# YuQiao0303/PointDreamer

Measured on AMD Instinct MI355X. Metric: shapes/hour (30k-pt cloud, 8x256^2 views, DDNM) on MI355X, higher is better.
Workload: dtype f16 (f32 accumulate; f32 GroupNorm/softmax statistics, f32 geometry); 1 GPU; configs[2]: synthetic 30k-point sphere shape, 8x256^2 views, texture_gen_method='DDNM_inpaint' (100 DDNM steps, 552.8M-param guided-diffusion UNet, random-init weights), NBF [21], atlas 1024^2, complete_unseen_by='unproject', optimize_from=None, hidden-point removal on (device); 4 independent shapes per step, their views batched through the UNet together; parallelism=shapes-parallel x1, views_per_unet_batch=32

## Files before the change

include/pdhip.h:

```cpp
#ifndef PDHIP_H
#define PDHIP_H
#include <stdint.h>
#include <stddef.h>
#ifdef __cplusplus
extern "C" {
#endif

#define PDHIP_OK 0
#define PDHIP_E_ARG (-1)
#define PDHIP_E_HIP (-2)
#define PDHIP_E_STATE (-3)
#define PDHIP_E_NOMEM (-4)
#define PDHIP_E_UNKNOWN_NAME (-5)

int pdhip_version(void);
int pdhip_lab_build(void);
const char* pdhip_last_error(void);

int pdhip_project_points(const float* cam_params, int V, const float* vertices, int Vn,
                         const float* points, int N, int rescale, double padding,
                         float* pos , float* vertice_uvs ,
                         float* uv_centers, float* uv_scales,
                         float* point_uvs , float* point_depths ,
                         uint32_t* minmax_ws, void* stream);
// ... 239 lines not shown
int pdhip_gn_finalize_oct_f32(const float* partA, int Ca, int chunksA, const float* partB, int Cb, int chunksB, int N, int HW, float* stats, void* stream);
int pdhip_conv_ht_f16(const void* x, const void* w_packed, const float* bias, const void* residual, int res_up, void* y, int N, int H, int W, int Cin, int Cout,
                      int Cout_pad, const void* zero_page, float* splitk_ws, long long splitk_ws_floats, float* gn_part, int* gn_chunks, void* stream);
int pdhip_conv_ht_plan(int N, int H, int W, int Cin, int Cout, int Cout_pad, long long splitk_ws_floats, int* routed, int* slabs);
int pdhip_debug_set_conv_ht(int mode, int slabs);
int pdhip_debug_set_rr_gn(int max_width);
int pdhip_debug_set_conv_rr(int mode, int variant, int slabs);
int pdhip_attention_f16(const void* qkv , void* out , int N, int T, int C, int head_dim,
                        void* vt_ws , void* stream);
int pdhip_philox_normal(float* out, long long n, uint64_t seed, uint64_t stream_id, void* stream);
int pdhip_gemv_rows_f32(const float* W, const float* b, const float* x, float* y, int R, int K, int N, int silu_out, void* stream);
int pdhip_timestep_mlp_f32(const float* t, int N, int mc, const float* w0, const float* b0, const float* w2, const float* b2, float* emb_silu,
                           float* tmp, void* stream);
int pdhip_conv_in_f16(const float* x_nchw, const void* Wt, const float* bias, void* Y, int N, int H, int W, int Cout, int Cout_pad, void* im2col_ws,
                      const void* zero_page, void* stream);
int pdhip_bench_copy16(const void* src, void* dst, long long bytes, int blocks, int unroll, void* stream);

#ifdef __cplusplus
}
#endif
#endif
```

pointdreamer_amd/csrc/nn_common.h:

```cpp
#pragma once
#include "common.h"
#include <hip/hip_fp16.h>

namespace pdnn {

typedef _Float16 half_t;
typedef __attribute__((ext_vector_type(8))) _Float16 half8;
typedef __attribute__((ext_vector_type(4))) _Float16 half4;
typedef __attribute__((ext_vector_type(4))) float float4_t;

bool conv3x3_halo_eligible(int N, int H, int W, int Cin, int Cout_pad);
int conv3x3_halo_splits(int N, int H, int W, int Cin, int Cout, int Cout_pad, size_t splitk_ws_floats);
int conv3x3_halo_launch_splits(int N, int H, int W, int Cin, int Cout, int Cout_pad, size_t halo_ws_floats);
int conv3x3_halo(const half_t* X, const half_t* Wt, const float* bias, const half_t* residual, half_t* Y, int N, int H, int W,
                 int Cin, int Cout, int Cout_pad, const half_t* zero_page, hipStream_t s, float* gn_part, int* gn_fused,
                 float* splitk_ws, size_t splitk_ws_floats, const float* apply_table = nullptr, int res_up = 0,
                 int in_up = 0);
int splitk_reduce(const float* partial, int splits, long long M, int Cout, const float* bias, const half_t* residual, half_t* Y,
                  float* gn_part, int hw, hipStream_t s);
extern thread_local int g_force_bk, g_force_stages, g_force_wmw, g_force_splits;
extern thread_local int g_fuse_gn, g_fold_resample, g_fold_finalize, g_fuse_skip, g_fold_skip;
extern thread_local float* g_dbg_splitk_ws; extern thread_local size_t g_dbg_splitk_floats;
int conv_igemm(const half_t* X, const half_t* Wt, const float* bias, const half_t* residual, half_t* Y, int N, int H,
               int W, int Cin, int Cout, int Cout_pad, int taps, const half_t* zero_page, hipStream_t s,
// ... 83 lines not shown
__device__ __forceinline__ float silu_f(float x) { return x * __builtin_amdgcn_rcpf(1.0f + __expf(-x)); }

__device__ __forceinline__ float gn_round_f16(float f) { asm("" : "+v"(f)); return (float)(half_t)f; }
template <bool OUT_F32, bool FILM>
__device__ __forceinline__ float gn_elem(float x, float ga, float gb, float t1, float sh, int silu) {
    float f = __builtin_fmaf(x, ga, gb);
    if (!OUT_F32) f = gn_round_f16(f);
    if (FILM) {
        f = gn_round_f16(f * t1);
        f = gn_round_f16(f + sh);
    }
    if (silu) { f = silu_f(f); if (!OUT_F32) f = gn_round_f16(f); }
    return f;
}


int gn_stats(const half_t* X, int N, int HW, int C, float eps, float* stats, float* ws, size_t ws_floats, hipStream_t s);
struct GnPartsArg { const float* partA; int Ca, chunksA; const float* partB; int Cb, chunksB; float eps; };
int gn_apply(const half_t* X, const float* stats, const float* gamma, const float* beta, const float* film,
             long long film_stride, int N, int H, int W, int C, int silu, int resample, void* Y, int out_f32, hipStream_t s,
             const half_t* XB = nullptr, int Ca = 0,
             half_t* Yraw = nullptr,
             const GnPartsArg* parts = nullptr);
int gn_table(const float* stats, const float* gamma, const float* beta, const float* film, long long film_stride, int N, int C,
             float* table, hipStream_t s);
bool gn_skip_eligible(int N, int HW, int Ca, int C, int Cout, int Cout_pad);
int gn_skip(const half_t* XA, const half_t* XB, int Ca, int C, const float* stats, const float* gamma, const float* beta, const half_t* Wt,
            const float* bias, half_t* H0, half_t* SK, int N, int HW, hipStream_t s);
int resample2x(const half_t* X, int N, int H, int W, int C, int mode, half_t* Y, hipStream_t s);
int concat_channels(const half_t* A, int Ca, const half_t* B, int Cb, long long pixels, half_t* Y, hipStream_t s);

int attention(const half_t* qkv, half_t* out, int N, int T, int C, int D, hipStream_t s, half_t* vt_ws = nullptr);

int conv_in_3x3(const float* x_nchw, const half_t* Wt , const float* bias, half_t* Y,
                int N, int H, int W, int Cout, int Cout_pad, half_t* im2col_ws , const half_t* zero_page, hipStream_t s, float* gn_part = nullptr, int* gn_fused = nullptr);
int head_pack(const float* w, int NO, int C, half_t* wz, hipStream_t s);
int head_gn_silu_conv3x3(const half_t* X, const float* stats, const float* gamma, const float* beta, const half_t* wz,
                         const float* bias, float* y_nchw, int N, int H, int W, int C, int NO, hipStream_t s);
int timestep_mlp(const float* t, int N, int mc, const float* w0, const float* b0, const float* w2, const float* b2,
                 float* emb_silu , float* tmp, hipStream_t s);
int gemv_rows(const float* Wm , const float* b, const float* x , float* y , int R, int K, int N,
              hipStream_t s);

struct DdnmCoef { float sqrt_1m_at, sqrt_at, sqrt_at_next, sigma_t, c1, c2; };
int ddnm_update(float* x , const float* et , int Cet, const float* y,
                const float* mask , const float* eps , unsigned long long seed,
                unsigned long long step, DdnmCoef co, int N, int HW, hipStream_t s, unsigned long long quad0 = 0);
int ddnm_prepare(const float* masked_img, const float* mask, float* y, int N, int HW, hipStream_t s);
int ddnm_finish(const float* x, float* out, long long n, hipStream_t s);
extern thread_local int g_gn_iters;
// ... 6 lines not shown
```

pointdreamer_amd/csrc/nn_misc.hip:

```cpp
#include "nn_common.h"
using namespace pdhip;
namespace pdnn {

__global__ __launch_bounds__(256) void k_im2col_in(const float* __restrict__ x, half_t* __restrict__ A, int H, int W,
                                                   long long pixels) {
    for (long long p = blockIdx.x * (long long)blockDim.x + threadIdx.x; p < pixels; p += (long long)gridDim.x * blockDim.x) {
        const int xx = (int)(p % W), y = (int)((p / W) % H);
        const long long n = p / ((long long)W * H);
        half_t row[32];
#pragma unroll
        for (int k = 27; k < 32; ++k) row[k] = (half_t)0.f;
#pragma unroll
        for (int ky = 0; ky < 3; ++ky)
#pragma unroll
            for (int kx = 0; kx < 3; ++kx) {
                const int yy = y + ky - 1, xc = xx + kx - 1;
                const bool ok = yy >= 0 && yy < H && xc >= 0 && xc < W;
#pragma unroll
                for (int c = 0; c < 3; ++c)
                    row[(ky * 3 + kx) * 3 + c] = ok ? (half_t)x[(((size_t)n * 3 + c) * H + yy) * W + xc] : (half_t)0.f;
            }
        half8* dst = reinterpret_cast<half8*>(A + (size_t)p * 32);
#pragma unroll
        for (int q = 0; q < 4; ++q) {
            half8 v;
#pragma unroll
            for (int e = 0; e < 8; ++e) v[e] = row[q * 8 + e];
            dst[q] = v;
        }
    }
}

int conv_in_3x3(const float* x_nchw, const half_t* Wt, const float* bias, half_t* Y, int N, int H, int W, int Cout, int Cout_pad,
                half_t* im2col_ws, const half_t* zero_page, hipStream_t s, float* gn_part, int* gn_fused) {
    const long long pixels = (long long)N * H * W;
    k_im2col_in<<<(int)std::min<long long>((pixels + 255) / 256, 8192), 256, 0, s>>>(x_nchw, im2col_ws, H, W, pixels);
    PD_LAUNCH_CHECK();
    return conv_igemm(im2col_ws, Wt, bias, nullptr, Y, N, H, W, 32, Cout, Cout_pad, 1, zero_page, s, nullptr, 0, gn_part, gn_fused);
}

#define GEMV_ROWS 128
template <int KI>
__global__ __launch_bounds__(256) void k_gemv_rows(const float* __restrict__ Wm, const float* __restrict__ b,
                                                   const float* __restrict__ x, float* __restrict__ y, int R, int K, int N,
                                                   int silu_out) {
    extern __shared__ __attribute__((aligned(16))) float s_x[];
    const int lane = threadIdx.x & 63, wave = threadIdx.x >> 6;
    const int r0 = blockIdx.x * GEMV_ROWS + wave * (GEMV_ROWS / 4);
    for (int n0 = 0; n0 < N; n0 += 8) {
        const int nb = min(8, N - n0);
// ... 239 lines not shown
    return pdnn::gemv_launch(W, b, x, y, R, K, N, silu_out != 0, as_stream(stream));
}
extern "C" int pdhip_timestep_mlp_f32(const float* t, int N, int mc, const float* w0, const float* b0, const float* w2, const float* b2,
                                      float* emb_silu, float* tmp, void* stream) {
    PD_REQUIRE(t && w0 && b0 && w2 && b2 && emb_silu && tmp, "pdhip_timestep_mlp_f32: null argument");
    PD_REQUIRE(N >= 1 && mc >= 2 && mc % 2 == 0 && mc <= 512, "pdhip_timestep_mlp_f32: N must be positive and mc even, at most 512 (N=%d mc=%d)", N, mc);
    return pdnn::timestep_mlp(t, N, mc, w0, b0, w2, b2, emb_silu, tmp, as_stream(stream));
}
extern "C" int pdhip_conv_in_f16(const float* x_nchw, const void* Wt, const float* bias, void* Y, int N, int H, int W, int Cout, int Cout_pad,
                                 void* im2col_ws, const void* zero_page, void* stream) {
    PD_REQUIRE(x_nchw && Wt && bias && Y && im2col_ws && zero_page, "pdhip_conv_in_f16: null argument");
    PD_REQUIRE(N >= 1 && H >= 1 && W >= 1 && Cout >= 1, "pdhip_conv_in_f16: N, H, W, Cout must be positive");
    return pdnn::conv_in_3x3(x_nchw, (const pdnn::half_t*)Wt, bias, (pdnn::half_t*)Y, N, H, W, Cout, Cout_pad, (pdnn::half_t*)im2col_ws, (const pdnn::half_t*)zero_page,
                             as_stream(stream), nullptr, nullptr);
}
```

pointdreamer_amd/csrc/nn_norm.hip:

```cpp
#include "nn_common.h"
using namespace pdhip;
namespace pdnn {

#define GN_PIX_PER_BLOCK 256

__global__ __launch_bounds__(256) void k_gn_partial(const half_t* __restrict__ X, int HW, int C, float* __restrict__ part) {
    extern __shared__ float s_acc[];
    const int n = blockIdx.y, chunk = blockIdx.x;
    const int opp = C >> 3;
    const int pps = max(1, 256 / opp);
    const int tid = threadIdx.x;
    const int sub = tid / opp, oct = tid - sub * opp;
    const int p0 = chunk * GN_PIX_PER_BLOCK;
    const int p1 = min(HW, p0 + GN_PIX_PER_BLOCK);
    float s[8], q[8];
#pragma unroll
    for (int e = 0; e < 8; ++e) { s[e] = 0.f; q[e] = 0.f; }
    if (sub < pps) {
        for (int oc = oct; oc < opp; oc += 256) {
            for (int p = p0 + sub; p < p1; p += pps) {
                const half8 v = *reinterpret_cast<const half8*>(X + ((size_t)n * HW + p) * C + oc * 8);
#pragma unroll
                for (int e = 0; e < 8; ++e) { const float f = (float)v[e]; s[e] += f; q[e] += f * f; }
            }
// ... 113 lines not shown
            float* row = table + ((size_t)n * (C / 8) + (c >> 3)) * 16;
            row[c & 7] = ga * t1; row[8 + (c & 7)] = gb * t1 + sh;
        }
    }
}
int gn_table(const float* stats, const float* gamma, const float* beta, const float* film, long long film_stride, int N, int C,
             float* table, hipStream_t s) {
    PD_REQUIRE(C % 32 == 0, "gn_table: C %% 32 != 0");
    k_gn_table<<<dim3(cdiv(C, 256), N), 256, 0, s>>>(stats, gamma, beta, film, film_stride, C, table);
    PD_LAUNCH_CHECK();
    return PDHIP_OK;
}


#define GNA_ITERS 8
struct GnParts { const float* a; const float* b; int Ca, Cb, chunksA, chunksB; float eps; };
template <int RES, bool OUT_F32, bool FILM, bool FIN>
__global__ __launch_bounds__(256) void k_gn_apply(const half_t* __restrict__ X, const float* __restrict__ stats,
                                                  const float* __restrict__ gamma, const float* __restrict__ beta,
                                                  const float* __restrict__ film, long long film_stride, int H, int W,
                                                  int C, int silu, void* __restrict__ Yv, const half_t* __restrict__ XB, int Ca, int iters,
                                                  half_t* __restrict__ Yraw, GnParts gp) {
    const int opp = C >> 3, cg = C / 32;
    const int pps = max(1, 256 / opp);
    const int Ho = RES == 1 ? H / 2 : (RES == 2 ? H * 2 : H), Wo = RES == 1 ? W / 2 : (RES == 2 ? W * 2 : W);
    __shared__ double s_fin[FIN ? 512 : 1];
    __shared__ float s_st[FIN ? 64 : 1];
    if (FIN) {
        const int img = blockIdx.y, fs = threadIdx.x / opp, fo = threadIdx.x - fs * opp;
        if (fs < pps) {
            const int oa = gp.Ca >> 3;
            const bool inA = fo < oa;
            const int chunks = inA ? gp.chunksA : gp.chunksB, os = inA ? oa : (gp.Cb >> 3);
            const float2* src = reinterpret_cast<const float2*>(inA ? gp.a : gp.b) + (size_t)img * chunks * os + (inA ? fo : fo - oa);
            double ds = 0.0, dq = 0.0;
#pragma unroll 8
            for (int c = fs; c < chunks; c += pps) { const float2 v = src[(size_t)c * os]; ds += (double)v.x; dq += (double)v.y; }
            s_fin[(fs * opp + fo) * 2] = ds; s_fin[(fs * opp + fo) * 2 + 1] = dq;
        }
        __syncthreads();
        if (threadIdx.x < 32) {
            const int opg = cg >> 3, g = threadIdx.x;
            double ds = 0.0, dq = 0.0;
            for (int k = 0; k < opg; ++k)
                for (int sl = 0; sl < pps; ++sl) { ds += s_fin[(sl * opp + g * opg + k) * 2]; dq += s_fin[(sl * opp + g * opg + k) * 2 + 1]; }
            const double cnt = (double)H * W * cg;
            const double mean = ds / cnt;
            double var = dq / cnt - mean * mean;
            if (var < 0.0) var = 0.0;
            s_st[2 * g] = (float)mean; s_st[2 * g + 1] = (float)(1.0 / sqrt(var + (double)gp.eps));
        }
        __syncthreads();
    }
#ifdef PD_LAB_GN_REV
    const int n = gridDim.y - 1 - blockIdx.y, bx = gridDim.x - 1 - blockIdx.x;
#else
    const int n = blockIdx.y, bx = blockIdx.x;
#endif
    const int sub = threadIdx.x / opp;
    if (sub >= pps) return;
    const int p_begin = bx * (pps * iters), p_end = min(Ho * Wo, p_begin + pps * iters);
    for (int oc = threadIdx.x - sub * opp; oc < opp; oc += 256) {
        const int c0 = oc * 8;
        const bool second = XB != nullptr && c0 >= Ca;
        const half_t* const Xs = second ? XB + (c0 - Ca) : X + c0;
        const int cs = XB == nullptr ? C : (second ? C - Ca : Ca);
        float ga[8], gb[8], t1[8], sh[8];
#pragma unroll
// ... 364 lines not shown
```

pointdreamer_amd/csrc/nn_unet.hip:

```cpp
#include "nn_common.h"
#include <map>
#include <string>
#include <vector>
#include <cmath>
#include <cstring>
using namespace pdhip;
using namespace pdnn;

namespace {

struct ConvW { half_t* w = nullptr; float* b = nullptr; int cin = 0, cout = 0, cout_pad = 0, taps = 0; bool have_w = false, have_b = false;
               half_t* wf = nullptr; half_t* wph = nullptr; bool has_wf = false, has_wph = false; };
struct NormW { float* g = nullptr; float* b = nullptr; int c = 0; bool have_g = false, have_b = false; };
struct ResB { std::string name; int cin, cout, mode; NormW n1, n2; ConvW c1, c2, skip; long long emb_off; bool has_skip; bool have_ew = false, have_eb = false;
              half_t* c2s_w = nullptr; float* c2s_b = nullptr; bool c2s_ready = false; half_t* c2s_wf = nullptr; int hw = 0; bool has_c2s = false, has_c2s_wf = false; };
struct AttB { std::string name; int c; NormW n; ConvW qkv, proj; };
struct Block { int kind; int idx; };

struct Act { half_t* p; int C, H, W; const float* gn_part = nullptr; int gn_chunks = 0; const float* gn_partB = nullptr; int Ca = 0; int gn_chunksB = 0;
             half_t* p2 = nullptr;
             int row = -1, rowB = -1; };

}
namespace pdnn { thread_local int g_fuse_gn = 0; }
namespace pdnn { thread_local int g_fold_resample = 1; }
namespace pdnn { thread_local int g_fold_skip = 1; }
namespace pdnn { thread_local int g_rr_gn = 0; }
namespace pdnn { thread_local int g_fold_finalize = 8; thread_local int g_fold_finalize_chunks = 16; }
namespace pdnn { thread_local int g_fuse_skip = 1; thread_local int g_fuse_skip_min_tiles = 1; }
namespace pdnn { thread_local int g_up_phase = 1; }
namespace {
struct Prof { std::vector<hipEvent_t> ev; std::vector<uint8_t> cls; size_t used = 0; double flops[2] = {0, 0}; bool on = false;
              int period = 1; long long forwards = 0; bool armed = false; };

}

// ... 188 lines not shown
}
ConvPlan plan_conv(const Ctx& c, const Act& x, const ConvW& w, bool want_gn) {
    ConvNeeds nd;
    nd.two_source = x.p2 != nullptr; nd.want_gn = want_gn; nd.have_wf = w.has_wf;
    return conv_plan(c.N, x.H, x.W, w.cin, w.cout, w.cout_pad, w.taps, nd, c.u->splitk_floats);
}

int run_gn_stats(Ctx& c, const Act& x) {
    if (x.gn_part != nullptr && ((x.C / 32) % 8) == 0)
        return gn_finalize_oct(x.gn_part, x.Ca, x.gn_chunks, x.gn_partB, x.C - x.Ca, x.gn_chunksB, c.N, x.H * x.W, 1e-5f, c.u->stats, c.s);
    PD_REQUIRE(x.p2 == nullptr, "unet: a virtual concat needs fused GroupNorm partials of both tensors");
    return gn_stats(x.p, c.N, x.H * x.W, x.C, 1e-5f, c.u->stats, c.u->gn_ws, c.u->gn_ws_floats, c.s);
}

int run_gn(Ctx& c, const Act& x, const NormW& n, const float* film, long long film_stride, int silu, int resample, Act* out,
           half_t* raw_pool = nullptr) {
    *out = Act{nullptr, x.C, 0, 0};
    out->H = resample == 1 ? x.H / 2 : (resample == 2 ? x.H * 2 : x.H);
    out->W = resample == 1 ? x.W / 2 : (resample == 2 ? x.W * 2 : x.W);
    out->p = arena_take(c.u, (size_t)c.N * out->H * out->W * x.C);
    if (!c.go()) return PDHIP_OK;
    PD_REQUIRE(n.have_g && n.have_b, "unet: norm weights not loaded");
#ifdef PD_LAB_SKIP_GN
    if (resample == 0 && x.p2 == nullptr && x.W <= 128 && silu) { out->p = x.p; return PDHIP_OK; }
#endif
    if (x.gn_part != nullptr && ((x.C / 32) % 8) == 0 && (x.C >> 3) <= 256 && g_fold_finalize > 0 &&
        (c.N <= g_fold_finalize || (x.gn_chunks <= g_fold_finalize_chunks && x.gn_chunksB <= g_fold_finalize_chunks))) {
        const GnPartsArg pa{x.gn_part, x.Ca, x.gn_chunks, x.gn_partB, x.C - x.Ca, x.gn_chunksB, 1e-5f};
        return gn_apply(x.p, nullptr, n.g, n.b, film, film_stride, c.N, x.H, x.W, x.C, silu, resample, out->p, 0, c.s, x.p2,
                        x.p2 ? x.Ca : 0, raw_pool, &pa);
    }
    PD_TRY(run_gn_stats(c, x));
    return gn_apply(x.p, c.u->stats, n.g, n.b, film, film_stride, c.N, x.H, x.W, x.C, silu, resample, out->p, 0, c.s, x.p2, x.p2 ? x.Ca : 0,
                    raw_pool);
}

int run_gn_then_conv(Ctx& c, const std::string& name, const ConvPlan& p, const Act& x, const NormW& n, const float* film, long long film_stride,
                     int resample, half_t* raw_pool, const ConvW& w, ConvIn in, Act* out) {
    if (p.takes_apply) {
        if (c.go()) {
            PD_REQUIRE(n.have_g && n.have_b, "unet: norm weights not loaded");
            PD_TRY(run_gn_stats(c, x));
            PD_TRY(gn_table(c.u->stats, n.g, n.b, film, film_stride, c.N, x.C, c.u->ap_table, c.s));
            in.apply_table = c.u->ap_table;
        }
        in.x = &x;
        return run_conv(c, name, p, w, in, out);
    }
    if (p.takes_in_gn) {
        if (c.go()) PD_REQUIRE(n.have_g && n.have_b, "unet: norm weights not loaded");
        const RrIn rr_in{x.p, nullptr, x.C, x.C, 2, n.g, n.b, film, film_stride, x.gn_part, nullptr, x.gn_chunks, 0, 1e-5f};
        in.x = &x; in.rr_in = &rr_in; in.parts_of = &x;
        return run_conv(c, name, p, w, in, out);
    }
    Act h;
    PD_TRY(run_gn(c, x, n, film, film_stride, 1, resample, &h, raw_pool));
    in.x = &h;
    if (x.p2 != nullptr) in.parts_of = &x;
    return run_conv(c, name, p, w, in, out);
}

struct ResPlan {
    bool fuse_skip = false;
    bool fold_down = false;
    bool fold_up = false;
    bool skip_conv = false;
    ConvPlan c1, c2, skip;
};
bool wish_in_gn(const Act& x, const ConvW& w, int W) {
    if (g_rr_gn <= 0 || W > g_rr_gn || x.p2 != nullptr || x.gn_part == nullptr || x.gn_partB != nullptr || ((x.C / 32) % 8) != 0 || w.cin > 1024 ||
        x.C != w.cin) return false;
    const int pps = std::max(1, 256 / (x.C >> 3));
    return (x.gn_chunks + pps - 1) / pps <= PD_RR_MAX_PART_LOADS;
}
bool wish_up_phase(int N, const ResB& rb, int H, int W) {
    if (g_up_phase == 0 || rb.mode != 2 || !rb.c1.has_wph || (H * W) % 256 != 0 ||
        !conv_up2_phase_eligible(N, H, W, rb.c1.cin, rb.c1.cout, rb.c1.cout_pad)) return false;
    if (g_up_phase == 2) return true;
    const long long tiles = (long long)N * H * W / 256 * 4 * (rb.c1.cout_pad / (rb.c1.cout_pad % 256 == 0 ? 256 : 128));
    return tiles >= 128;
}
// ... 3 lines not shown
    const bool lean = !conservative;
    const bool fold = g_fold_resample != 0 && lean && x.p2 == nullptr && !rb.has_skip;
    r.fold_down = fold && rb.mode == 1;
    r.fuse_skip = rb.has_skip && rb.mode == 0 && g_fuse_skip != 0 && rb.skip.taps == 1 && x.C == rb.skip.cin &&
                  gn_skip_eligible(N, x.H * x.W, x.p2 ? x.Ca : x.C, x.C, rb.skip.cout, rb.skip.cout_pad) &&
                  (g_fuse_skip == 2 || (long long)N * x.H * x.W / 128 >= g_fuse_skip_min_tiles) &&
                  (conservative || (x.gn_part != nullptr && ((x.C / 32) % 8) == 0));
    ConvNeeds n1;
    n1.want_gn = true; n1.have_wf = rb.c1.has_wf;
    if (lean && !r.fuse_skip && rb.mode == 0 && x.p2 == nullptr) { n1.apply = g_fuse_gn != 0; n1.in_gn = wish_in_gn(x, rb.c1, x.W); }
    n1.in_up = fold && rb.mode == 2;
    if (lean && x.p2 == nullptr && !rb.has_skip && wish_up_phase(N, rb, x.H, x.W))
        r.c1 = conv_up2_phase_plan(N, Ho, Wo, rb.c1.cin, rb.c1.cout, rb.c1.cout_pad, true);
    else
        r.c1 = conv_plan(N, Ho, Wo, rb.c1.cin, rb.c1.cout, rb.c1.cout_pad, 9, n1, ws_floats);
    Act h1{nullptr, rb.cout, Ho, Wo};
    if (r.c1.gn_chunks > 0) { h1.gn_part = x.gn_part ? x.gn_part : reinterpret_cast<const float*>(&r); h1.gn_chunks = r.c1.gn_chunks; h1.Ca = rb.cout; }
    ConvNeeds n2;
    n2.want_gn = true; n2.have_wf = rb.c2.has_wf;
    if (lean) { n2.apply = g_fuse_gn != 0; n2.in_gn = wish_in_gn(h1, rb.c2, Wo); }
    if (lean && rb.has_skip && !r.fuse_skip && g_fold_skip != 0 && rb.mode == 0 && rb.has_c2s && rb.skip.taps == 1 &&
        (x.p2 == nullptr || (x.Ca % 64 == 0 && (x.C - x.Ca) % 64 == 0))) {
        n2.skip_cs = rb.skip.cin;
        n2.have_wf_skip = rb.has_c2s_wf && (x.p2 == nullptr || (x.Ca % 128 == 0 && (x.C - x.Ca) % 128 == 0));
    }
    r.c2 = conv_plan(N, Ho, Wo, rb.c2.cin, rb.c2.cout, rb.c2.cout_pad, 9, n2, ws_floats);
    r.fold_up = fold && rb.mode == 2 && r.c2.takes_res_up;
    r.skip_conv = rb.has_skip && !r.fuse_skip && !r.c2.takes_skip;
    if (r.skip_conv) {
        ConvNeeds ns;
// ... 16 lines not shown
    if (r.fuse_skip) {
        Act h0{nullptr, x.C, x.H, x.W};
        h0.p = arena_take(c.u, (size_t)c.N * x.H * x.W * x.C);
        sk = Act{nullptr, rb.skip.cout, x.H, x.W};
        sk.p = arena_take(c.u, (size_t)c.N * x.H * x.W * rb.skip.cout);
        if (c.go()) {
            PD_REQUIRE(rb.n1.have_g && rb.n1.have_b && rb.skip.have_w && rb.skip.have_b, "unet: norm / skip weights of %s not loaded", rb.name.c_str());
            PD_TRY(run_gn_stats(c, x));
            PD_TRY(gn_skip(x.p, x.p2, x.p2 ? x.Ca : x.C, x.C, c.u->stats, rb.n1.g, rb.n1.b, rb.skip.w, rb.skip.b, h0.p, sk.p, c.N, x.H * x.W, c.s));
        }
        ConvIn in{&h0};
        in.parts_of = &x; in.note = "gn_skip";
        PD_TRY(run_conv(c, n1, r.c1, rb.c1, in, &h1));
    } else {
        const bool half_res = r.c1.kernel == CONV_UP_PHASE || r.c1.takes_in_up;
        PD_TRY(run_gn_then_conv(c, n1, r.c1, x, rb.n1, nullptr, 0, half_res ? 0 : rb.mode, r.fold_down ? xr.p : nullptr, rb.c1, ConvIn{nullptr}, &h1));
    }
    if (rb.mode != 0 && c.go() && !r.fold_down && !r.fold_up) PD_TRY(resample2x(x.p, c.N, x.H, x.W, x.C, rb.mode, xr.p, c.s));
    if (!r.fuse_skip) sk = r.fold_up ? x : xr;
    if (r.skip_conv) PD_TRY(run_conv(c, rb.name + ".skip_connection", r.skip, rb.skip, ConvIn{&xr}, &sk));
    ConvIn in2{nullptr, r.c2.takes_skip ? nullptr : sk.p, r.fold_up ? 1 : 0};
    in2.skip_src = &x; in2.skip_w = &rb;
    return run_gn_then_conv(c, rb.name + ".out_layers.3", r.c2, h1, rb.n2, film, c.film_stride, 0, nullptr, rb.c2, in2, out);
}

int run_att(Ctx& c, const Act& x, AttB& ab, Act* out) {
    Act xn, qkv, a;
    PD_TRY(run_gn(c, x, ab.n, nullptr, 0, 0, 0, &xn));
    PD_TRY(run_conv(c, ab.name + ".qkv", plan_conv(c, xn, ab.qkv, false), ab.qkv, ConvIn{&xn}, &qkv));
    a = x;
    a.p = arena_take(c.u, (size_t)c.N * x.H * x.W * x.C);
    half_t* vt = arena_take(c.u, (size_t)c.N * x.H * x.W * x.C);
    if (c.go()) {
        const double T = (double)x.H * x.W;
        PD_TRY(prof_begin(c, 4.0 * c.N * T * T * x.C, 1));
        PD_TRY(attention(qkv.p, a.p, c.N, x.H * x.W, x.C, c.u->head, c.s, vt));
        PD_TRY(prof_end(c));
    }
    return run_conv(c, ab.name + ".proj_out", plan_conv(c, a, ab.proj, true), ab.proj, ConvIn{&a, x.p}, out);
}

int run_blocks(Ctx& c, std::vector<Block>& blocks, Act* h, const float* x_nchw) {
    for (Block& b : blocks) {
        Act o;
        if (b.kind == 0) {
            o.C = c.u->mult[0] * c.u->mc; o.H = o.W = c.u->image_size;
            const int cpad = ((o.C + 127) / 128) * 128;
            ConvNeeds nd;
            nd.want_gn = true;
            const ConvPlan p = conv_plan(c.N, o.H, o.W, 32, o.C, cpad, 1, nd, 0);
            o.p = arena_take(c.u, (size_t)c.N * o.H * o.W * o.C);
            half_t* col = arena_take(c.u, (size_t)c.N * o.H * o.W * 32);
            float* part = reinterpret_cast<float*>(arena_take(c.u, (size_t)c.N * ((o.H * o.W + 127) / 128) * (o.C / 8) * 2 * 2));
            if (c.table) { Act in{nullptr, 32, o.H, o.W}; table_row(c, "input_blocks.0.0", p, ConvIn{&in}, &o); adopt_parts(&o, part, p.gn_chunks); }
            if (c.go()) {
                PD_REQUIRE(c.u->have_win && c.u->have_bin, "unet: input conv not loaded");
                int chunks = 0;
                PD_TRY(conv_in_3x3(x_nchw, c.u->w_in, c.u->b_in, o.p, c.N, o.H, o.W, o.C, cpad, col, c.u->zero_page, c.s, part, &chunks));
                PD_REQUIRE(chunks == p.gn_chunks, "unet: input conv: planned for %d partial chunks per image, the launcher left %d", p.gn_chunks, chunks);
                adopt_parts(&o, part, chunks);
            }
// ... 553 lines not shown
    int old = pdnn::g_sk_mode;
    pdnn::g_sk_mode = mode; pdnn::g_sk_tile = tile; pdnn::g_sk_splits = splits;
    return old;
}
extern "C" int pdhip_debug_set_conv_sk_stages(int stages) { int old = pdnn::g_sk_stages; pdnn::g_sk_stages = stages; return old; }
extern "C" int pdhip_debug_set_conv_sk_kgroups(int kg) { int old = pdnn::g_sk_kg; pdnn::g_sk_kg = kg; return old; }
namespace pdnn { extern thread_local int g_attn_nbuf, g_attn_vt, g_attn_qtn; }
extern "C" int pdhip_debug_set_attn(int nbuf, int vt_form, int qtiles) {
    int old = pdnn::g_attn_nbuf | (pdnn::g_attn_vt << 8) | (pdnn::g_attn_qtn << 16);
    pdnn::g_attn_nbuf = nbuf; pdnn::g_attn_vt = vt_form; pdnn::g_attn_qtn = qtiles;
    return old;
}
extern "C" int pdhip_debug_set_conv_sk_order(int order) { int old = pdnn::g_sk_order; pdnn::g_sk_order = order; return old; }
extern "C" int pdhip_debug_set_rr_gn(int max_width) { int old = pdnn::g_rr_gn; pdnn::g_rr_gn = max_width; return old; }
extern "C" int pdhip_debug_set_up_phase(int mode) { int old = pdnn::g_up_phase; pdnn::g_up_phase = mode; return old; }
extern "C" int pdhip_pack_conv_up2_phase_f16(const void* w_packed, int Cin, int Cout_pad, void* w_phase, void* stream) {
    PD_REQUIRE(w_packed && w_phase && Cin > 0 && Cout_pad > 0, "pdhip_pack_conv_up2_phase_f16: bad arguments");
    return conv_up2_phase_pack((const half_t*)w_packed, Cin, Cout_pad, (half_t*)w_phase, as_stream(stream));
}
extern "C" int pdhip_conv3x3_up2_phase_nhwc_f16(const void* x, const void* w_phase, const float* bias, void* y, int N, int H, int W, int Cin, int Cout,
                                                int Cout_pad, const void* zero_page, float* gn_part, void* stream) {
    PD_REQUIRE(x && w_phase && y && zero_page, "pdhip_conv3x3_up2_phase_nhwc_f16: null argument");
    return conv_up2_phase((const half_t*)x, (const half_t*)w_phase, bias, (half_t*)y, N, H, W, Cin, Cout, Cout_pad, (const half_t*)zero_page,
                          as_stream(stream), gn_part, nullptr);
}
extern "C" int pdhip_conv3x3_up2_halo_nhwc_f16(const void* x, const void* w_packed, const float* bias, void* y, int N, int H, int W, int Cin, int Cout,
                                               int Cout_pad, const void* zero_page, void* stream) {
    PD_REQUIRE(x && w_packed && y && zero_page, "pdhip_conv3x3_up2_halo_nhwc_f16: null argument");
    pdnn::ConvNeeds nd;
    nd.in_up = true;
// ... 95 lines not shown
```

pointdreamer_amd/ddnm_inpainting.py:

```python
import ctypes as C
import math
import os

import torch

from . import _lib
from ._lib import ptr, stream, check

_reg = _lib.register
vp, i32, i64, f32, f64, u64 = C.c_void_p, C.c_int, C.c_int64, C.c_float, C.c_double, C.c_uint64
_reg('pdhip_unet_create', C.c_int, [i32, i32, i32, C.POINTER(C.c_int), i32, C.POINTER(C.c_int), i32, i32, i32, i32,
                                    C.POINTER(vp)])
_reg('pdhip_unet_destroy', None, [vp])
_reg('pdhip_unet_arena_bytes', C.c_longlong, [vp])
_reg('pdhip_unet_num_tensors', C.c_int, [vp])
_reg('pdhip_unet_load_tensor', C.c_int, [vp, C.c_char_p, vp, i32, C.POINTER(C.c_int64), i32, vp])
_reg('pdhip_unet_missing_tensors', C.c_int, [vp, C.c_char_p, i32])
_reg('pdhip_unet_forward', C.c_int, [vp, vp, vp, i32, vp, vp])
_reg('pdhip_unet_profile', C.c_int, [vp, i32])
_reg('pdhip_unet_profile_read', C.c_int, [vp, C.POINTER(C.c_double), C.POINTER(C.c_double), C.POINTER(C.c_longlong)])
_reg('pdhip_unet_profile_read_attention', C.c_int, [vp, C.POINTER(C.c_double), C.POINTER(C.c_double), C.POINTER(C.c_longlong)])
_reg('pdhip_ddnm_schedule', C.c_int, [vp, vp, vp, vp, vp])
_reg('pdhip_ddnm_prepare', C.c_int, [vp, vp, vp, i32, i32, vp])
_reg('pdhip_ddnm_step', C.c_int, [vp, vp, i32, vp, vp, vp, u64, i32, i32, i32, vp])
# ... 36 lines not shown
_reg('pdhip_conv_rr_weight_halfs', C.c_longlong, [i32, i32, i32, i32])
_reg('pdhip_conv_rr_pack_f16', C.c_int, [vp, i32, i32, i32, i32, vp, vp])
_reg('pdhip_gn_octet_partials_f16', C.c_int, [vp, i32, i32, i32, i32, vp, vp])
_reg('pdhip_gn_apply_parts_f16', C.c_int, [vp, vp, i32, i32, vp, i32, vp, i32, vp, vp, vp, C.c_longlong, i32, i32, i32, i32, vp, vp])
_reg('pdhip_conv_rr_f16', C.c_int, [vp, vp, i32, i32, i32, vp, vp, vp, C.c_longlong, vp, i32, vp, i32, vp, vp, i32, i32, i32, vp, vp, vp, i32, vp,
                                   i32, i32, i32, i32, vp, C.c_longlong, vp, C.POINTER(C.c_int), vp])
_reg('pdhip_debug_conv_launch_nhwc_f16', C.c_int, [vp, vp, i32, vp, vp, vp, i32, vp, vp, i32, i32, vp, i32, i32, i32, i32, i32, i32, i32, vp, vp, C.c_longlong,
                                                  vp, C.c_longlong, C.POINTER(C.c_int), C.POINTER(C.c_int), vp])
_reg('pdhip_gn_finalize_oct_f32', C.c_int, [vp, i32, i32, vp, i32, i32, i32, i32, vp, vp])
_reg('pdhip_debug_conv3x3_apply', C.c_int, [vp, vp, vp, vp, vp, vp, i32, i32, i32, i32, i32, i32, vp, vp])
_reg('pdhip_attention_f16', C.c_int, [vp, vp, i32, i32, i32, i32, vp, vp])
_reg('pdhip_philox_normal', C.c_int, [vp, C.c_longlong, u64, u64, vp])
_reg('pdhip_gemv_rows_f32', C.c_int, [vp, vp, vp, vp, i32, i32, i32, i32, vp])
_reg('pdhip_timestep_mlp_f32', C.c_int, [vp, i32, i32, vp, vp, vp, vp, vp, vp, vp])
_reg('pdhip_conv_in_f16', C.c_int, [vp, vp, vp, vp, i32, i32, i32, i32, i32, vp, vp, vp])
_reg('pdhip_debug_set_gn_iters', C.c_int, [i32])
_reg('pdhip_bench_copy16', C.c_int, [vp, vp, C.c_longlong, i32, i32, vp])

IMAGENET_256 = dict(image_size=256, num_channels=256, num_res_blocks=2, attention_resolutions="32,16,8",
                    num_head_channels=64, learn_sigma=True, use_scale_shift_norm=True, resblock_updown=True,
                    use_fp16=True, channel_mult="")
DEFAULT_CKPT = 'models/DDNM/256x256_diffusion_uncond.pt'


def default_channel_mult(image_size):
    return {512: (0.5, 1, 1, 2, 2, 4, 4), 256: (1, 1, 2, 2, 4, 4), 128: (1, 1, 2, 3, 4), 64: (1, 2, 3, 4)}[image_size]


def unet_route_table(N, image_size=256, num_channels=256, num_res_blocks=2, attention_resolutions="32,16,8", num_head_channels=64,
                     learn_sigma=True, channel_mult="", max_batch=64, **unused):
# ... 209 lines not shown
```

Measured before the change: 2077 shapes/hour.

## Add direct MFMA input conv and recompute it fused with first GroupNorm+SiLU

Replaces the im2col plus generic implicit-GEMM input convolution with a direct kernel that builds the 27-tap patch in LDS, runs MFMA and emits GroupNorm partials. For the first resblock's GN+SiLU, it recomputes the cheap 3-channel input conv, folding in the statistics finalize, instead of re-reading the 256-channel full-resolution activation. This trades extra MFMA work and re-reading the small input for less HBM traffic and fewer launches. The shared GN finalize logic is moved into a common device helper.

```diff
diff --git a/include/pdhip.h b/include/pdhip.h
--- a/include/pdhip.h
+++ b/include/pdhip.h
@@ -277,6 +277,12 @@
                            float* tmp, void* stream);
 int pdhip_conv_in_f16(const float* x_nchw, const void* Wt, const float* bias, void* Y, int N, int H, int W, int Cout, int Cout_pad, void* im2col_ws,
                       const void* zero_page, void* stream);
+int pdhip_debug_set_unet_ends(int on);
+int pdhip_debug_conv_in_f16(const float* x_nchw, const void* Wt, const float* bias, void* Y, int N, int H, int W, int Cout, int Cout_pad, void* im2col_ws,
+                            const void* zero_page, float* gn_part, long long gn_part_floats, int* gn_chunks, void* stream);
+int pdhip_debug_conv_in_tile(int N, int H, int W, int Cout, int Cout_pad);
+int pdhip_debug_conv_in_gn_silu_f16(const float* x_nchw, const void* Wt, const float* bias, void* Yn, int N, int H, int W, int Cout, int Cout_pad,
+                                    const float* gn_part, int gn_chunks, const float* stats, const float* gamma, const float* beta, void* stream);
 int pdhip_bench_copy16(const void* src, void* dst, long long bytes, int blocks, int unroll, void* stream);
 
 #ifdef __cplusplus
diff --git a/pointdreamer_amd/csrc/nn_common.h b/pointdreamer_amd/csrc/nn_common.h
--- a/pointdreamer_amd/csrc/nn_common.h
+++ b/pointdreamer_amd/csrc/nn_common.h
@@ -121,6 +121,36 @@
     return f;
 }
 
+struct GnParts { const float* a; const float* b; int Ca, Cb, chunksA, chunksB; float eps; };
+__device__ __forceinline__ void gn_fin_stats(const GnParts& gp, int img, int H, int W, int C, double* s_fin, float* s_st) {
+    const int opp = C >> 3, cg = C / 32;
+    const int pps = max(1, 256 / opp);
+    const int fs = threadIdx.x / opp, fo = threadIdx.x - fs * opp;
+    if (fs < pps) {
+        const int oa = gp.Ca >> 3;
+        const bool inA = fo < oa;
+        const int chunks = inA ? gp.chunksA : gp.chunksB, os = inA ? oa : (gp.Cb >> 3);
+        const float2* src = reinterpret_cast<const float2*>(inA ? gp.a : gp.b) + (size_t)img * chunks * os + (inA ? fo : fo - oa);
+        double ds = 0.0, dq = 0.0;
+#pragma unroll 8
+        for (int c = fs; c < chunks; c += pps) { const float2 v = src[(size_t)c * os]; ds += (double)v.x; dq += (double)v.y; }
+        s_fin[(fs * opp + fo) * 2] = ds; s_fin[(fs * opp + fo) * 2 + 1] = dq;
+    }
+    __syncthreads();
+    if (threadIdx.x < 32) {
+        const int opg = cg >> 3, g = threadIdx.x;
+        double ds = 0.0, dq = 0.0;
+        for (int k = 0; k < opg; ++k)
+            for (int sl = 0; sl < pps; ++sl) { ds += s_fin[(sl * opp + g * opg + k) * 2]; dq += s_fin[(sl * opp + g * opg + k) * 2 + 1]; }
+        const double cnt = (double)H * W * cg;
+        const double mean = ds / cnt;
+        double var = dq / cnt - mean * mean;
+        if (var < 0.0) var = 0.0;
+        s_st[2 * g] = (float)mean; s_st[2 * g + 1] = (float)(1.0 / sqrt(var + (double)gp.eps));
+    }
+    __syncthreads();
+}
+
 
 int gn_stats(const half_t* X, int N, int HW, int C, float eps, float* stats, float* ws, size_t ws_floats, hipStream_t s);
 struct GnPartsArg { const float* partA; int Ca, chunksA; const float* partB; int Cb, chunksB; float eps; };
@@ -141,6 +171,10 @@
 
 int conv_in_3x3(const float* x_nchw, const half_t* Wt , const float* bias, half_t* Y,
                 int N, int H, int W, int Cout, int Cout_pad, half_t* im2col_ws , const half_t* zero_page, hipStream_t s, float* gn_part = nullptr, int* gn_fused = nullptr);
+extern thread_local int g_unet_ends;
+int conv_in_direct_tile(int N, int H, int W, int Cout, int Cout_pad);
+int conv_in_gn_silu(const float* x_nchw, const half_t* Wt, const float* bias, half_t* Yn, int N, int H, int W, int Cout, int Cout_pad,
+                    const float* stats, const GnPartsArg* parts, const float* gamma, const float* beta, hipStream_t s);
 int head_pack(const float* w, int NO, int C, half_t* wz, hipStream_t s);
 int head_gn_silu_conv3x3(const half_t* X, const float* stats, const float* gamma, const float* beta, const half_t* wz,
                          const float* bias, float* y_nchw, int N, int H, int W, int C, int NO, hipStream_t s);
diff --git a/pointdreamer_amd/csrc/nn_misc.hip b/pointdreamer_amd/csrc/nn_misc.hip
--- a/pointdreamer_amd/csrc/nn_misc.hip
+++ b/pointdreamer_amd/csrc/nn_misc.hip
@@ -31,9 +31,151 @@
     }
 }
 
+template <int BMT, int MODE, bool FIN>
+__global__ __launch_bounds__(256) void k_conv_in(const float* __restrict__ x, const half_t* __restrict__ Wt, const float* __restrict__ bias,
+                                                 half_t* __restrict__ Y, int H, int W, int Cout, float* __restrict__ gn_part,
+                                                 const float* __restrict__ stats, const float* __restrict__ gamma, const float* __restrict__ beta, GnParts gp) {
+    __shared__ half8 As[4 * BMT];
+    __shared__ float red[MODE == 0 ? 16 * 64 * 2 : 1];
+    __shared__ double s_fin[FIN ? 512 : 1];
+    __shared__ float s_st[FIN ? 64 : 1];
+    const int tid = threadIdx.x, lane = tid & 63, wave = tid >> 6, r16 = lane & 15, q = lane >> 4;
+    const int hw = H * W;
+    const long long m0 = (long long)blockIdx.x * BMT;
+    const int img = (int)(m0 / hw), rem0 = (int)(m0 - (long long)img * hw);
+    if (FIN) gn_fin_stats(gp, img, H, W, Cout, s_fin, s_st);
+    const float* const xi = x + (size_t)img * 3 * hw;
+#pragma unroll
+    for (int it = 0; it < 4 * BMT / 256; ++it) {
+        const int idx = it * 256 + tid, p = idx % BMT, kc = idx / BMT;
+        const int rem = rem0 + p, py = rem / W, px = rem - py * W;
+        half8 v;
+#pragma unroll
+        for (int e = 0; e < 8; ++e) {
+            const int k = kc * 8 + e, tap = k / 3, c = k - tap * 3, ky = tap / 3, kx = tap - ky * 3;
+            const int yy = py + ky - 1, xc = px + kx - 1;
+            const bool ok = k < 27 && yy >= 0 && yy < H && xc >= 0 && xc < W;
+            v[e] = ok ? (half_t)xi[(c * H + yy) * W + xc] : (half_t)0.f;
+        }
+        As[kc * BMT + p] = v;
+    }
+    __syncthreads();
+    for (int cg = wave; cg * 64 < Cout; cg += 4) {
+        const int c_lo = cg * 64 + q * 8, c_hi = c_lo + 32;
+        const bool ok_lo = c_lo < Cout, ok_hi = c_hi < Cout;
+        half8 wf[4];
+#pragma unroll
+        for (int j = 0; j < 4; ++j)
+            wf[j] = *reinterpret_cast<const half8*>(Wt + (size_t)(cg * 64 + (j >> 1) * 32 + (r16 >> 2) * 8 + (j & 1) * 4 + (r16 & 3)) * 32 + q * 8);
+        float bv[16];
+#pragma unroll
+        for (int e = 0; e < 8; ++e) { bv[e] = ok_lo ? bias[c_lo + e] : 0.f; bv[8 + e] = ok_hi ? bias[c_hi + e] : 0.f; }
+        float ga[MODE == 1 ? 16 : 1], gb[MODE == 1 ? 16 : 1];
+        if (MODE == 1) {
+            const int cgs = Cout / 32;
+#pragma unroll
+            for (int e = 0; e < 16; ++e) {
+                const int c = (e < 8 ? c_lo : c_hi - 8) + e, grp = min(c, Cout - 1) / cgs;
+                const float mean = FIN ? s_st[2 * grp] : stats[((size_t)img * 32 + grp) * 2], rstd = FIN ? s_st[2 * grp + 1] : stats[((size_t)img * 32 + grp) * 2 + 1];
+                ga[e] = rstd * gamma[min(c, Cout - 1)];
+                gb[e] = beta[min(c, Cout - 1)] - mean * ga[e];
+            }
+        }
+        float gs0 = 0.f, gq0 = 0.f, gs1 = 0.f, gq1 = 0.f;
+#pragma unroll 2
+        for (int i = 0; i < BMT / 16; ++i) {
+            const half8 b = As[q * BMT + i * 16 + r16];
+            float4_t acc[4];
+#pragma unroll
+            for (int j = 0; j < 4; ++j) acc[j] = __builtin_amdgcn_mfma_f32_16x16x32_f16(wf[j], b, (float4_t){0.f, 0.f, 0.f, 0.f}, 0, 0, 0);
+            half8 lo, hi;
+#pragma unroll
+            for (int r = 0; r < 4; ++r) {
+                lo[r] = (half_t)(acc[0][r] + bv[r]); lo[4 + r] = (half_t)(acc[1][r] + bv[4 + r]);
+                hi[r] = (half_t)(acc[2][r] + bv[8 + r]); hi[4 + r] = (half_t)(acc[3][r] + bv[12 + r]);
+            }
+            half_t* const dst = Y + (size_t)(m0 + i * 16 + r16) * Cout;
+            if (MODE == 0) {
+                if (ok_lo) {
+                    *reinterpret_cast<half8*>(dst + c_lo) = lo;
+#pragma unroll
+                    for (int e = 0; e < 8; ++e) { const float f = (float)lo[e]; gs0 += f; gq0 += f * f; }
+                }
+                if (ok_hi) {
+                    *reinterpret_cast<half8*>(dst + c_hi) = hi;
+#pragma unroll
+                    for (int e = 0; e < 8; ++e) { const float f = (float)hi[e]; gs1 += f; gq1 += f * f; }
+                }
+            } else {
+                half8 nlo, nhi;
+#pragma unroll
+                for (int e = 0; e < 8; ++e) {
+                    nlo[e] = (half_t)gn_elem<false, false>((float)lo[e], ga[e], gb[e], 1.f, 0.f, 1);
+                    nhi[e] = (half_t)gn_elem<false, false>((float)hi[e], ga[8 + e], gb[8 + e], 1.f, 0.f, 1);
+                }
+                if (ok_lo) *reinterpret_cast<half8*>(dst + c_lo) = nlo;
+                if (ok_hi) *reinterpret_cast<half8*>(dst + c_hi) = nhi;
+            }
+        }
+        if (MODE == 0 && gn_part != nullptr) {
+            if (ok_lo) { red[(r16 * 64 + (c_lo >> 3)) * 2] = gs0; red[(r16 * 64 + (c_lo >> 3)) * 2 + 1] = gq0; }
+            if (ok_hi) { red[(r16 * 64 + (c_hi >> 3)) * 2] = gs1; red[(r16 * 64 + (c_hi >> 3)) * 2 + 1] = gq1; }
+        }
+    }
+    if (MODE == 0 && gn_part != nullptr) {
+        __syncthreads();
+        const int chunks = hw / BMT, chunk = rem0 / BMT;
+        for (int o = tid; o < (Cout >> 3); o += 256) {
+            float s1 = 0.f, q1 = 0.f;
+            for (int r = 0; r < 16; ++r) { s1 += red[(r * 64 + o) * 2]; q1 += red[(r * 64 + o) * 2 + 1]; }
+            float* dst = gn_part + (((size_t)img * chunks + chunk) * (Cout >> 3) + o) * 2;
+            dst[0] = s1; dst[1] = q1;
+        }
+    }
+}
+
+thread_local int g_unet_ends = 1;
+
+int conv_in_direct_tile(int N, int H, int W, int Cout, int Cout_pad) {
+    if (g_unet_ends == 0 || Cout % 8 != 0 || Cout > 512 || Cout_pad % 128 != 0 || Cout_pad < Cout) return 0;
+    ConvNeeds nd;
+    nd.want_gn = true;
+    const ConvPlan p = conv_plan(N, H, W, 32, Cout, Cout_pad, 1, nd, 0);
+    if (p.kernel != CONV_IGEMM || p.splits != 1 || (p.geo != 2 && p.geo != 8)) return 0;
+    const int bmt = p.geo == 2 ? 128 : 256;
+    return ((long long)H * W) % bmt == 0 ? bmt : 0;
+}
+
+int conv_in_gn_silu(const float* x_nchw, const half_t* Wt, const float* bias, half_t* Yn, int N, int H, int W, int Cout, int Cout_pad,
+                    const float* stats, const GnPartsArg* parts, const float* gamma, const float* beta, hipStream_t s) {
+    const int bmt = conv_in_direct_tile(N, H, W, Cout, Cout_pad);
+    PD_REQUIRE(bmt != 0 && Cout % 32 == 0 && ((Cout / 32) % 8) == 0, "conv_in_gn_silu: not a shape the recompute form takes (N=%d H=%d W=%d Cout=%d)", N, H, W, Cout);
+    PD_REQUIRE((stats != nullptr) != (parts != nullptr), "conv_in_gn_silu: pass finished statistics or the conv's partials, not both");
+    PD_REQUIRE(parts == nullptr || (parts->partA != nullptr && parts->Ca == Cout && parts->Cb == 0 && parts->chunksA > 0),
+               "conv_in_gn_silu: the partials must be those of the input conv alone");
+    GnParts gp{nullptr, nullptr, 0, 0, 0, 0, 0.f};
+    if (parts != nullptr) gp = GnParts{parts->partA, nullptr, parts->Ca, 0, parts->chunksA, 0, parts->eps};
+    const unsigned grid = (unsigned)((long long)N * H * W / bmt);
+#define CIN_GN(B_) do { if (parts) k_conv_in<B_, 1, true><<<grid, 256, 0, s>>>(x_nchw, Wt, bias, Yn, H, W, Cout, nullptr, nullptr, gamma, beta, gp); \
+                        else k_conv_in<B_, 1, false><<<grid, 256, 0, s>>>(x_nchw, Wt, bias, Yn, H, W, Cout, nullptr, stats, gamma, beta, gp); } while (0)
+    if (bmt == 128) CIN_GN(128); else CIN_GN(256);
+#undef CIN_GN
+    PD_LAUNCH_CHECK();
+    return PDHIP_OK;
+}
+
 int conv_in_3x3(const float* x_nchw, const half_t* Wt, const float* bias, half_t* Y, int N, int H, int W, int Cout, int Cout_pad,
                 half_t* im2col_ws, const half_t* zero_page, hipStream_t s, float* gn_part, int* gn_fused) {
     const long long pixels = (long long)N * H * W;
+    if (const int bmt = conv_in_direct_tile(N, H, W, Cout, Cout_pad)) {
+        const GnParts none{nullptr, nullptr, 0, 0, 0, 0, 0.f};
+        const unsigned grid = (unsigned)(pixels / bmt);
+        if (bmt == 128) k_conv_in<128, 0, false><<<grid, 256, 0, s>>>(x_nchw, Wt, bias, Y, H, W, Cout, gn_part, nullptr, nullptr, nullptr, none);
+        else k_conv_in<256, 0, false><<<grid, 256, 0, s>>>(x_nchw, Wt, bias, Y, H, W, Cout, gn_part, nullptr, nullptr, nullptr, none);
+        PD_LAUNCH_CHECK();
+        if (gn_fused) *gn_fused = gn_part != nullptr ? (int)(((long long)H * W) / bmt) : 0;
+        return PDHIP_OK;
+    }
     k_im2col_in<<<(int)std::min<long long>((pixels + 255) / 256, 8192), 256, 0, s>>>(x_nchw, im2col_ws, H, W, pixels);
     PD_LAUNCH_CHECK();
     return conv_igemm(im2col_ws, Wt, bias, nullptr, Y, N, H, W, 32, Cout, Cout_pad, 1, zero_page, s, nullptr, 0, gn_part, gn_fused);
@@ -303,3 +445,20 @@
     return pdnn::conv_in_3x3(x_nchw, (const pdnn::half_t*)Wt, bias, (pdnn::half_t*)Y, N, H, W, Cout, Cout_pad, (pdnn::half_t*)im2col_ws, (const pdnn::half_t*)zero_page,
                              as_stream(stream), nullptr, nullptr);
 }
+extern "C" int pdhip_debug_conv_in_f16(const float* x_nchw, const void* Wt, const float* bias, void* Y, int N, int H, int W, int Cout, int Cout_pad,
+                                       void* im2col_ws, const void* zero_page, float* gn_part, long long gn_part_floats, int* gn_chunks, void* stream) {
+    PD_REQUIRE(x_nchw && Wt && bias && Y && im2col_ws && zero_page && gn_part && gn_chunks, "pdhip_debug_conv_in_f16: null argument");
+    PD_REQUIRE(N >= 1 && H >= 1 && W >= 1 && Cout >= 1, "pdhip_debug_conv_in_f16: N, H, W, Cout must be positive");
+    PD_REQUIRE(gn_part_floats >= (long long)N * (((long long)H * W + 127) / 128) * (Cout / 8) * 2, "pdhip_debug_conv_in_f16: gn_part is too small for 128-pixel chunks");
+    return pdnn::conv_in_3x3(x_nchw, (const pdnn::half_t*)Wt, bias, (pdnn::half_t*)Y, N, H, W, Cout, Cout_pad, (pdnn::half_t*)im2col_ws, (const pdnn::half_t*)zero_page,
+                             as_stream(stream), gn_part, gn_chunks);
+}
+extern "C" int pdhip_debug_conv_in_tile(int N, int H, int W, int Cout, int Cout_pad) { return pdnn::conv_in_direct_tile(N, H, W, Cout, Cout_pad); }
+extern "C" int pdhip_debug_conv_in_gn_silu_f16(const float* x_nchw, const void* Wt, const float* bias, void* Yn, int N, int H, int W, int Cout, int Cout_pad,
+                                               const float* gn_part, int gn_chunks, const float* stats, const float* gamma, const float* beta, void* stream) {
+    PD_REQUIRE(x_nchw && Wt && bias && Yn && gamma && beta, "pdhip_debug_conv_in_gn_silu_f16: null argument");
+    PD_REQUIRE(N >= 1 && H >= 1 && W >= 1 && Cout >= 1, "pdhip_debug_conv_in_gn_silu_f16: N, H, W, Cout must be positive");
+    const pdnn::GnPartsArg pa{gn_part, Cout, gn_chunks, nullptr, 0, 0, 1e-5f};
+    return pdnn::conv_in_gn_silu(x_nchw, (const pdnn::half_t*)Wt, bias, (pdnn::half_t*)Yn, N, H, W, Cout, Cout_pad, stats, gn_part ? &pa : nullptr, gamma, beta,
+                                 as_stream(stream));
+}
diff --git a/pointdreamer_amd/csrc/nn_norm.hip b/pointdreamer_amd/csrc/nn_norm.hip
--- a/pointdreamer_amd/csrc/nn_norm.hip
+++ b/pointdreamer_amd/csrc/nn_norm.hip
@@ -151,7 +151,6 @@
 
 
 #define GNA_ITERS 8
-struct GnParts { const float* a; const float* b; int Ca, Cb, chunksA, chunksB; float eps; };
 template <int RES, bool OUT_F32, bool FILM, bool FIN>
 __global__ __launch_bounds__(256) void k_gn_apply(const half_t* __restrict__ X, const float* __restrict__ stats,
                                                   const float* __restrict__ gamma, const float* __restrict__ beta,
@@ -163,32 +162,7 @@
     const int Ho = RES == 1 ? H / 2 : (RES == 2 ? H * 2 : H), Wo = RES == 1 ? W / 2 : (RES == 2 ? W * 2 : W);
     __shared__ double s_fin[FIN ? 512 : 1];
     __shared__ float s_st[FIN ? 64 : 1];
-    if (FIN) {
-        const int img = blockIdx.y, fs = threadIdx.x / opp, fo = threadIdx.x - fs * opp;
-        if (fs < pps) {
-            const int oa = gp.Ca >> 3;
-            const bool inA = fo < oa;
-            const int chunks = inA ? gp.chunksA : gp.chunksB, os = inA ? oa : (gp.Cb >> 3);
-            const float2* src = reinterpret_cast<const float2*>(inA ? gp.a : gp.b) + (size_t)img * chunks * os + (inA ? fo : fo - oa);
-            double ds = 0.0, dq = 0.0;
-#pragma unroll 8
-            for (int c = fs; c < chunks; c += pps) { const float2 v = src[(size_t)c * os]; ds += (double)v.x; dq += (double)v.y; }
-            s_fin[(fs * opp + fo) * 2] = ds; s_fin[(fs * opp + fo) * 2 + 1] = dq;
-        }
-        __syncthreads();
-        if (threadIdx.x < 32) {
-            const int opg = cg >> 3, g = threadIdx.x;
-            double ds = 0.0, dq = 0.0;
-            for (int k = 0; k < opg; ++k)
-                for (int sl = 0; sl < pps; ++sl) { ds += s_fin[(sl * opp + g * opg + k) * 2]; dq += s_fin[(sl * opp + g * opg + k) * 2 + 1]; }
-            const double cnt = (double)H * W * cg;
-            const double mean = ds / cnt;
-            double var = dq / cnt - mean * mean;
-            if (var < 0.0) var = 0.0;
-            s_st[2 * g] = (float)mean; s_st[2 * g + 1] = (float)(1.0 / sqrt(var + (double)gp.eps));
-        }
-        __syncthreads();
-    }
+    if (FIN) gn_fin_stats(gp, blockIdx.y, H, W, C, s_fin, s_st);
 #ifdef PD_LAB_GN_REV
     const int n = gridDim.y - 1 - blockIdx.y, bx = gridDim.x - 1 - blockIdx.x;
 #else
diff --git a/pointdreamer_amd/csrc/nn_unet.hip b/pointdreamer_amd/csrc/nn_unet.hip
--- a/pointdreamer_amd/csrc/nn_unet.hip
+++ b/pointdreamer_amd/csrc/nn_unet.hip
@@ -19,7 +19,8 @@
 
 struct Act { half_t* p; int C, H, W; const float* gn_part = nullptr; int gn_chunks = 0; const float* gn_partB = nullptr; int Ca = 0; int gn_chunksB = 0;
              half_t* p2 = nullptr;
-             int row = -1, rowB = -1; };
+             int row = -1, rowB = -1;
+             bool from_conv_in = false; const float* conv_in_x = nullptr; };
 
 }
 namespace pdnn { thread_local int g_fuse_gn = 0; }
@@ -238,7 +239,7 @@
 }
 
 int run_gn(Ctx& c, const Act& x, const NormW& n, const float* film, long long film_stride, int silu, int resample, Act* out,
-           half_t* raw_pool = nullptr) {
+           half_t* raw_pool = nullptr, bool recompute_in = false) {
     *out = Act{nullptr, x.C, 0, 0};
     out->H = resample == 1 ? x.H / 2 : (resample == 2 ? x.H * 2 : x.H);
     out->W = resample == 1 ? x.W / 2 : (resample == 2 ? x.W * 2 : x.W);
@@ -251,16 +252,20 @@
     if (x.gn_part != nullptr && ((x.C / 32) % 8) == 0 && (x.C >> 3) <= 256 && g_fold_finalize > 0 &&
         (c.N <= g_fold_finalize || (x.gn_chunks <= g_fold_finalize_chunks && x.gn_chunksB <= g_fold_finalize_chunks))) {
         const GnPartsArg pa{x.gn_part, x.Ca, x.gn_chunks, x.gn_partB, x.C - x.Ca, x.gn_chunksB, 1e-5f};
+        if (recompute_in)
+            return conv_in_gn_silu(x.conv_in_x, c.u->w_in, c.u->b_in, out->p, c.N, x.H, x.W, x.C, ((x.C + 127) / 128) * 128, nullptr, &pa, n.g, n.b, c.s);
         return gn_apply(x.p, nullptr, n.g, n.b, film, film_stride, c.N, x.H, x.W, x.C, silu, resample, out->p, 0, c.s, x.p2,
                         x.p2 ? x.Ca : 0, raw_pool, &pa);
     }
     PD_TRY(run_gn_stats(c, x));
+    if (recompute_in)
+        return conv_in_gn_silu(x.conv_in_x, c.u->w_in, c.u->b_in, out->p, c.N, x.H, x.W, x.C, ((x.C + 127) / 128) * 128, c.u->stats, nullptr, n.g, n.b, c.s);
     return gn_apply(x.p, c.u->stats, n.g, n.b, film, film_stride, c.N, x.H, x.W, x.C, silu, resample, out->p, 0, c.s, x.p2, x.p2 ? x.Ca : 0,
                     raw_pool);
 }
 
 int run_gn_then_conv(Ctx& c, const std::string& name, const ConvPlan& p, const Act& x, const NormW& n, const float* film, long long film_stride,
-                     int resample, half_t* raw_pool, const ConvW& w, ConvIn in, Act* out) {
+                     int resample, half_t* raw_pool, const ConvW& w, ConvIn in, Act* out, bool recompute_in = false) {
     if (p.takes_apply) {
         if (c.go()) {
             PD_REQUIRE(n.have_g && n.have_b, "unet: norm weights not loaded");
@@ -278,7 +283,7 @@
         return run_conv(c, name, p, w, in, out);
     }
     Act h;
-    PD_TRY(run_gn(c, x, n, film, film_stride, 1, resample, &h, raw_pool));
+    PD_TRY(run_gn(c, x, n, film, film_stride, 1, resample, &h, raw_pool, recompute_in));
     in.x = &h;
     if (x.p2 != nullptr) in.parts_of = &x;
     return run_conv(c, name, p, w, in, out);
@@ -289,6 +294,7 @@
     bool fold_down = false;
     bool fold_up = false;
     bool skip_conv = false;
+    bool recompute_in = false;
     ConvPlan c1, c2, skip;
 };
 bool wish_in_gn(const Act& x, const ConvW& w, int W) {
@@ -322,6 +328,9 @@
         r.c1 = conv_up2_phase_plan(N, Ho, Wo, rb.c1.cin, rb.c1.cout, rb.c1.cout_pad, true);
     else
         r.c1 = conv_plan(N, Ho, Wo, rb.c1.cin, rb.c1.cout, rb.c1.cout_pad, 9, n1, ws_floats);
+    r.recompute_in = lean && g_unet_ends != 0 && x.from_conv_in && rb.mode == 0 && !r.fuse_skip && x.p2 == nullptr && x.gn_part != nullptr && x.gn_partB == nullptr &&
+                     x.C % 32 == 0 && ((x.C / 32) % 8) == 0 && (x.C >> 3) <= 256 && !r.c1.takes_apply && !r.c1.takes_in_gn &&
+                     conv_in_direct_tile(N, x.H, x.W, x.C, ((x.C + 127) / 128) * 128) != 0;
     Act h1{nullptr, rb.cout, Ho, Wo};
     if (r.c1.gn_chunks > 0) { h1.gn_part = x.gn_part ? x.gn_part : reinterpret_cast<const float*>(&r); h1.gn_chunks = r.c1.gn_chunks; h1.Ca = rb.cout; }
     ConvNeeds n2;
@@ -368,7 +377,8 @@
         PD_TRY(run_conv(c, n1, r.c1, rb.c1, in, &h1));
     } else {
         const bool half_res = r.c1.kernel == CONV_UP_PHASE || r.c1.takes_in_up;
-        PD_TRY(run_gn_then_conv(c, n1, r.c1, x, rb.n1, nullptr, 0, half_res ? 0 : rb.mode, r.fold_down ? xr.p : nullptr, rb.c1, ConvIn{nullptr}, &h1));
+        PD_TRY(run_gn_then_conv(c, n1, r.c1, x, rb.n1, nullptr, 0, half_res ? 0 : rb.mode, r.fold_down ? xr.p : nullptr, rb.c1, ConvIn{nullptr}, &h1,
+                                r.recompute_in));
     }
     if (rb.mode != 0 && c.go() && !r.fold_down && !r.fold_up) PD_TRY(resample2x(x.p, c.N, x.H, x.W, x.C, rb.mode, xr.p, c.s));
     if (!r.fuse_skip) sk = r.fold_up ? x : xr;
@@ -399,6 +409,7 @@
         Act o;
         if (b.kind == 0) {
             o.C = c.u->mult[0] * c.u->mc; o.H = o.W = c.u->image_size;
+            o.from_conv_in = true; o.conv_in_x = x_nchw;
             const int cpad = ((o.C + 127) / 128) * 128;
             ConvNeeds nd;
             nd.want_gn = true;
@@ -982,6 +993,7 @@
 extern "C" int pdhip_debug_set_conv_sk_order(int order) { int old = pdnn::g_sk_order; pdnn::g_sk_order = order; return old; }
 extern "C" int pdhip_debug_set_rr_gn(int max_width) { int old = pdnn::g_rr_gn; pdnn::g_rr_gn = max_width; return old; }
 extern "C" int pdhip_debug_set_up_phase(int mode) { int old = pdnn::g_up_phase; pdnn::g_up_phase = mode; return old; }
+extern "C" int pdhip_debug_set_unet_ends(int on) { int old = pdnn::g_unet_ends; pdnn::g_unet_ends = on; return old; }
 extern "C" int pdhip_pack_conv_up2_phase_f16(const void* w_packed, int Cin, int Cout_pad, void* w_phase, void* stream) {
     PD_REQUIRE(w_packed && w_phase && Cin > 0 && Cout_pad > 0, "pdhip_pack_conv_up2_phase_f16: bad arguments");
     return conv_up2_phase_pack((const half_t*)w_packed, Cin, Cout_pad, (half_t*)w_phase, as_stream(stream));
diff --git a/pointdreamer_amd/ddnm_inpainting.py b/pointdreamer_amd/ddnm_inpainting.py
--- a/pointdreamer_amd/ddnm_inpainting.py
+++ b/pointdreamer_amd/ddnm_inpainting.py
@@ -74,6 +74,10 @@
 _reg('pdhip_gemv_rows_f32', C.c_int, [vp, vp, vp, vp, i32, i32, i32, i32, vp])
 _reg('pdhip_timestep_mlp_f32', C.c_int, [vp, i32, i32, vp, vp, vp, vp, vp, vp, vp])
 _reg('pdhip_conv_in_f16', C.c_int, [vp, vp, vp, vp, i32, i32, i32, i32, i32, vp, vp, vp])
+_reg('pdhip_debug_set_unet_ends', C.c_int, [i32])
+_reg('pdhip_debug_conv_in_f16', C.c_int, [vp, vp, vp, vp, i32, i32, i32, i32, i32, vp, vp, vp, C.c_longlong, C.POINTER(C.c_int), vp])
+_reg('pdhip_debug_conv_in_tile', C.c_int, [i32, i32, i32, i32, i32])
+_reg('pdhip_debug_conv_in_gn_silu_f16', C.c_int, [vp, vp, vp, vp, i32, i32, i32, i32, i32, vp, i32, vp, vp, vp, vp])
 _reg('pdhip_debug_set_gn_iters', C.c_int, [i32])
 _reg('pdhip_bench_copy16', C.c_int, [vp, vp, C.c_longlong, i32, i32, vp])
 
```

Result: no change. 2083 shapes/hour, median of 6 (+0.3%).
